# andreeaiana/manner

Measured on AMD Instinct MI355X. Metric: candidate news encoded+scored/sec, higher is better.
Workload: dtype f16; 1 GPU; configs[1]: CR-Module late fusion, MIND-small shape (65238-news pool), bert-base-uncased architectu~; modules=1, parallelism=dp1 (impressions sharded, no collective)

## Files before the change

### manner_amd/build.py

```python
from __future__ import annotations

import os
import subprocess
import sys
from concurrent.futures import ThreadPoolExecutor

PKG = os.path.dirname(os.path.abspath(__file__))
ROOT = os.path.dirname(PKG)
CSRC = os.path.join(PKG, "csrc")
LIB = os.path.join(PKG, "lib", "libmanner_hip.so")
SOURCES = ["gemm.hip", "rowops.hip", "attention.hip", "attention_d32.hip", "scoring.hip", "pool.hip", "entity.hip", "metrics.hip", "collate.hip", "cache.hip", "encoder.hip", "train.hip", "train_attn.hip", "wgrad.hip", "train_small.hip", "axis0.hip", "rows_f32.hip", "poly.hip", "caum.hip", "gru.hip", "mins.hip", "miner.hip", "aspect.hip", "debias.hip", "seqcls.hip", "tsne.hip"]
FLAGS = ["--offload-arch=gfx950", "-O3", "-std=c++17", "-fPIC", "-fno-gpu-rdc", "-Wall", "-Wno-unused-function",
         "-I" + os.path.join(ROOT, "include"), "-I" + CSRC]


def _newest(paths):
    return max(os.path.getmtime(p) for p in paths)


def build_library(force: bool = False, verbose: bool = True) -> str:
    hipcc = os.environ.get("HIPCC", "/opt/rocm/bin/hipcc")
    objdir = os.path.join(PKG, "lib", "obj")
    os.makedirs(objdir, exist_ok=True)
    if not all(os.path.exists(os.path.join(CSRC, f"gemm_w{nw}_asm.inc")) for nw in (8, 4)):
        subprocess.run([sys.executable, os.path.join(ROOT, "tools", "gen_gemm_w.py")], check=True, capture_output=True)
    headers = [os.path.join(CSRC, "common.h"), os.path.join(CSRC, "train_common.h"), os.path.join(CSRC, "row_head.h"), os.path.join(CSRC, "gemm_w4_asm.inc"), os.path.join(CSRC, "gemm_w8_asm.inc"), os.path.join(ROOT, "include", "manner_hip.h")]
    if not force and os.path.exists(LIB) and os.path.getmtime(LIB) >= _newest([os.path.join(CSRC, s) for s in SOURCES] + headers):
        return LIB
    jobs = []
    for s in SOURCES:
        src, obj = os.path.join(CSRC, s), os.path.join(objdir, s + ".o")
        if force or not os.path.exists(obj) or os.path.getmtime(obj) < _newest([src] + headers):
            jobs.append((src, obj))

    def cc(job):
        src, obj = job
        cmd = [hipcc] + FLAGS + ["-c", src, "-o", obj]
        r = subprocess.run(cmd, capture_output=True, text=True)
        return job, r

    with ThreadPoolExecutor(max_workers=min(4, max(1, len(jobs)))) as ex:
        for (src, obj), r in ex.map(cc, jobs):
            if verbose and (r.stdout or r.stderr):
                sys.stderr.write(r.stdout + r.stderr)
            if r.returncode:
                raise RuntimeError(f"hipcc failed on {src}")
    objs = [os.path.join(objdir, s + ".o") for s in SOURCES]
    if jobs or not os.path.exists(LIB):
        r = subprocess.run([hipcc, "--offload-arch=gfx950", "-shared", "-fPIC", "-o", LIB] + objs,
                           capture_output=True, text=True)
        if r.returncode:
            sys.stderr.write(r.stdout + r.stderr)
            raise RuntimeError("link of libmanner_hip.so failed")
    return LIB


if __name__ == "__main__":
    print(build_library(force="--force" in sys.argv))
```

### manner_amd/csrc/common.h

```cpp
#pragma once
#include <hip/hip_runtime.h>
#include <stddef.h>
#include <stdint.h>

#include "manner_hip.h"

typedef __bf16 bf16_t;
typedef __bf16 bf16x8 __attribute__((ext_vector_type(8)));
typedef __bf16 bf16x4 __attribute__((ext_vector_type(4)));
typedef _Float16 f16_t;
typedef _Float16 f16x8 __attribute__((ext_vector_type(8)));
typedef _Float16 f16x4 __attribute__((ext_vector_type(4)));
typedef short s16x4 __attribute__((ext_vector_type(4)));
typedef float f32x16 __attribute__((ext_vector_type(16)));
typedef float f32x4 __attribute__((ext_vector_type(4)));

#define LDS_PTR(p) ((__attribute__((address_space(3))) void*)(p))
#define GLOBAL_PTR(p) ((const __attribute__((address_space(1))) void*)(p))

namespace manner {

int fail(int code, const char* fmt, ...);

#define MANNER_HIP_TRY(expr)                                                            \
// ... 52 lines not shown
                EPI_GELU_GRAD = 9 ,
                EPI_BIAS_GELU_DUAL16 = 10 ,
                EPI_GELU_GRAD16 = 11  };
enum DType { DT_F32 = 0, DT_BF16 = 1, DT_F16 = 2 };
static inline bool is_16bit(DType d) { return d != DT_F32; }

template <typename T> struct E16;
template <> struct E16<bf16_t> {
  typedef bf16x8 v8; typedef bf16x4 v4;
  static constexpr DType dtype = DT_BF16;
  static __device__ __forceinline__ f32x4 mfma16(const v8& a, const v8& b, const f32x4& c) { return __builtin_amdgcn_mfma_f32_16x16x32_bf16(a, b, c, 0, 0, 0); }
  static __device__ __forceinline__ f32x16 mfma32(const v8& a, const v8& b, const f32x16& c) { return __builtin_amdgcn_mfma_f32_32x32x16_bf16(a, b, c, 0, 0, 0); }
};
template <> struct E16<f16_t> {
  typedef f16x8 v8; typedef f16x4 v4;
  static constexpr DType dtype = DT_F16;
  static __device__ __forceinline__ f32x4 mfma16(const v8& a, const v8& b, const f32x4& c) { return __builtin_amdgcn_mfma_f32_16x16x32_f16(a, b, c, 0, 0, 0); }
  static __device__ __forceinline__ f32x16 mfma32(const v8& a, const v8& b, const f32x16& c) { return __builtin_amdgcn_mfma_f32_32x32x16_f16(a, b, c, 0, 0, 0); }
};

int gemm_tn(DType in, DType out, Epilogue epi, const void* X, const void* W, const float* bias,
            const void* residual, void* Y, int64_t m_bound, int N, int K, const int* m_total,
            hipStream_t stream);

int gemm_tn_batched16(DType in, const void* X, const void* W, const float* bias, float* Y, int batch, int64_t xs, int64_t ws,
                      int64_t ys, int rows, int N, int K, const int* m_total, hipStream_t stream);

struct DlnFinalize { void* mr_out; int32_t* arrive; float eps; bool done; };
int gemm_tn_dln(DType dt, Epilogue epi, const void* X, const void* W, const float* bias, const float* vec, const void* mr,
                void* part, void* Y, int64_t m_bound, int N, int K, const int* m_total, hipStream_t stream, int64_t m_exact = -1,
                DlnFinalize* fin = nullptr);

int pool_logits_mfma(const float* x, const float* W, const float* bias, const float* query, int64_t R, int D, int Q,
                     float* logits, hipStream_t stream);

bool pool_fused_supported(int64_t B, int64_t S, int D, int Q);
size_t pool_fused_workspace_bytes(int D, int Q);
int pool_fused(const float* x, const float* W, const float* bias, const float* query, int64_t B, int64_t S, int D, int Q, float* out,
               void* workspace, size_t workspace_bytes, hipStream_t stream);

int lengths_and_offsets(const int64_t* mask, int64_t n_news, int64_t padded_len, int32_t* lens,
                        int32_t* cu , int32_t* m_total , int64_t m_bound,
                        int64_t expect_tokens, int32_t* status, hipStream_t stream, int max_len);
int embed_layernorm(DType out, const int64_t* ids, int64_t n_news, int64_t padded_len, const int32_t* cu,
                    const float* word, const float* pos, const float* type0, const float* gamma,
                    const float* beta, int H, float eps, int pos_offset, int vocab, int max_pos,
                    void* x, int32_t* status, hipStream_t stream);
int layernorm_rows(DType out, const float* pre, const float* gamma, const float* beta, int H, float eps,
                   void* x, int64_t m_bound, const int* m_total, hipStream_t stream);
int embed_raw(DType dt, const int64_t* ids, int64_t n_news, int64_t padded_len, const int32_t* cu, const float* word,
              const float* pos, const float* type0, int H, float eps, int pos_offset, int vocab, int max_pos,
              void* raw, void* mr, int32_t* status, hipStream_t stream);
__device__ __forceinline__ float2 dln_row_stats(const float2 (&v)[16], float inv_h, float eps) {
  float s1 = v[0].x, s2 = v[0].y;
#pragma unroll
  for (int g = 1; g < 16; ++g) { s1 += v[g].x; s2 += v[g].y; }
  const float mean = s1 * inv_h;
  const float var = fmaxf(fmaf(s2, inv_h, -(mean * mean)), 0.f);
  return float2{mean, 1.0f / sqrtf(var + eps)};
}
int dln_finalize(const void* part, int groups, int H, float eps, void* mr, int64_t m_bound, const int* m_total,
                 hipStream_t stream);
int gather_cls_ln(DType dt, const void* raw, const void* mr, const int32_t* cu, int64_t n_news, int H, const float* gamma,
                  const float* beta, void* dst, hipStream_t stream);
int fold_layernorm(DType dt, const float* w, const float* bias, const float* gamma, const float* beta, int N, int K, void* wf,
                   float* c1, float* c2, hipStream_t stream);
int scatter_hidden(DType in, DType out_dt, const void* x, const void* mr, const int32_t* cu, int64_t n_news, int64_t lp, int H,
                   const float* gamma, const float* beta, void* out, hipStream_t stream);
int split3_rows(DType dt, bool weight, const float* x, void* out, int K, int64_t rows, const int* m_total, hipStream_t stream);
int layernorm_rows_split(DType split_dt, const float* pre, const float* gamma, const float* beta, int H, float eps, float* x, void* a3,
                         int64_t m_bound, const int* m_total, hipStream_t stream);
int add_vectors(const float* a, const float* b, float* out, int n, hipStream_t stream);
int set_device_int(int32_t* p, int32_t value, hipStream_t stream);
int gather_cls(DType in, const void* x, const int32_t* cu, int64_t n_news, int H, float* out, hipStream_t stream);
int gather_cls_rows(DType dt, const void* x, const int32_t* cu, int64_t n_news, int H, void* dst, hipStream_t stream);
int convert_f32_to_16(DType dt, const float* src, void* dst, int64_t n, hipStream_t stream);

int attention_varlen(DType dt, const void* qkv, void* ctx, const int32_t* cu, int64_t n_news, int heads,
                     int H, int max_len, hipStream_t stream, void* split_out = nullptr, DType split_dt = DT_F32);

int attention_cls(DType dt, const void* qcls, const void* kv, void* ctx_cls, const int32_t* cu, int64_t n_news,
                  int heads, int H, hipStream_t stream);

int attention_varlen_d32(DType dt, const void* qkv, void* ctx, const int32_t* cu, int64_t n_news, int heads, int H, int max_len,
                         hipStream_t stream);
int attention_cls_d32(DType dt, const void* qcls, const void* kv, void* ctx_cls, const int32_t* cu, int64_t n_news, int heads, int H,
                      hipStream_t stream);

int launch_axis0_attention(const float* qkv, float* att, int64_t N, int64_t E, int D, int heads, bool train_tiles, hipStream_t stream);

int wlin_f32(bool tanh_act, const float* x, int ldx, const float* W, int ldw, const float* bias, int64_t R, int K, int O, float* y, int ldy,
             hipStream_t stream);
int wlin_dx_f32(const float* dy, int ldy, const float* W, int ldw, int64_t R, int K, int O, float* dx, float* wt, hipStream_t stream);

constexpr int LIN_ROWS_OT = 64;
int launch_lin_rows(bool tanh_act, const float* x, const float* W, int ldw, const float* b, const float* rowadd, int S, int64_t R, int K, int O, float* y,
                    int ldy, float* deriv, hipStream_t stream);
int launch_proj_rows(const float* x, int64_t xsb, int64_t xss, const int64_t* len, const float* W, const float* b, int S, int C, int64_t R, int K, int O,
                     float* gi, float* xs, hipStream_t stream);
int launch_dx_rows(const float* dy, int ldy, const float* W, int ldw, int64_t R, int K, int O, const float* add, const float* mul, float* dx,
                   hipStream_t stream);
constexpr int WGRAD_MAX_GROUPS = 16, WGRAD_GROUP_ROWS = 64;
int wgrad_rows_groups(int64_t R);
size_t wgrad_rows_part_floats(int64_t R, int K, int O);
int launch_wgrad_rows(const float* dy, int ldy, const float* x, int64_t R, int K, int O, float* part, float* dW, int ldo, hipStream_t stream);
int launch_wgrad_reduce(const float* part, int K, int O, int G, float* dW, int ldo, hipStream_t stream);
int launch_colsum_rows(const float* dy, int ldy, int64_t R, int O, float* db, hipStream_t stream);
int launch_transpose_tile(const float* in, int ldw, int O, int K, float* out, hipStream_t stream);

struct FloatBump {
  float* base;
  size_t off = 0;
  explicit FloatBump(void* p) : base(static_cast<float*>(p)) {}
  float* take(size_t n) {
    float* p = base ? base + off : nullptr;
    off += (n + 63) / 64 * 64;
    return p;
  }
};

}
```

### manner_amd/csrc/encoder.hip

```cpp
#include <stdarg.h>
#include <stdio.h>
#include <stdlib.h>

#include <vector>

#include "common.h"

namespace manner {

static thread_local char g_err[512] = "";

int fail(int code, const char* fmt, ...) {
  va_list ap;
  va_start(ap, fmt);
  vsnprintf(g_err, sizeof(g_err), fmt, ap);
  va_end(ap);
  return code;
}

struct LayerWeights {
  void* wqkv = nullptr;
  void* wo = nullptr;
  void* w1 = nullptr;
  void* w2 = nullptr;
  void* wqkv_f = nullptr;
  void* w1_f = nullptr;
  float *cq1 = nullptr, *cf1 = nullptr;
};
struct LayerParams {
  float *bqkv, *bo, *ln1g, *ln1b, *b1, *b2, *ln2g, *ln2b;
  float *cq2 = nullptr, *cf2 = nullptr, *bo_res = nullptr, *b2_res = nullptr;
};

}

struct manner_hip_encoder {
  manner_hip_encoder_config cfg;
  uint32_t precisions = 0;
  float *word = nullptr, *pos = nullptr, *type0 = nullptr, *embg = nullptr, *embb = nullptr;
  std::vector<manner::LayerParams> params;
  std::vector<manner::LayerWeights> w[5];
  int32_t* status = nullptr;
  static constexpr int ARRIVE_CAP = 4096;
  int32_t* arrive = nullptr;
  std::vector<void*> allocs;
  int n_streams = 2;
  bool defer_ln = false;
  static constexpr int MAX_STREAMS = 4;
  hipStream_t side[MAX_STREAMS] = {};
  hipEvent_t join_ev[MAX_STREAMS] = {};
  hipEvent_t phase_ev[MAX_STREAMS] = {};
  bool profiling = false;
  struct Span { hipEvent_t a, b; int cls; };
  std::vector<Span> spans;
  std::vector<hipEvent_t> free_events;
};

namespace manner {
namespace {

inline DType act_dtype(int prec) { return prec == MANNER_HIP_PREC_BF16 ? DT_BF16 : prec == MANNER_HIP_PREC_F16 ? DT_F16 : DT_F32; }
inline size_t act_bytes(int prec) { return (prec == MANNER_HIP_PREC_BF16 || prec == MANNER_HIP_PREC_F16) ? 2 : 4; }
inline bool is_x3(int prec) { return prec == MANNER_HIP_PREC_BF16X3 || prec == MANNER_HIP_PREC_F16X3; }
inline DType x3_dtype(int prec) { return prec == MANNER_HIP_PREC_F16X3 ? DT_F16 : DT_BF16; }

int dev_alloc(manner_hip_encoder* e, size_t bytes, void** out) {
  MANNER_HIP_TRY(hipMalloc(out, bytes));
  e->allocs.push_back(*out);
  return MANNER_HIP_OK;
}
int dev_copy_f32(manner_hip_encoder* e, const float* src, size_t n, float** out, hipStream_t s) {
  int rc = dev_alloc(e, n * sizeof(float), (void**)out);
  if (rc) return rc;
  MANNER_HIP_TRY(hipMemcpyAsync(*out, src, n * sizeof(float), hipMemcpyDeviceToDevice, s));
  return MANNER_HIP_OK;
}
int pack_matrix(int prec, const float* src, size_t n, void* dst, size_t elem_off, hipStream_t s) {
  if (prec == MANNER_HIP_PREC_BF16 || prec == MANNER_HIP_PREC_F16)
    return convert_f32_to_16(prec == MANNER_HIP_PREC_F16 ? DT_F16 : DT_BF16, src, static_cast<char*>(dst) + elem_off * 2, (int64_t)n, s);
  MANNER_HIP_TRY(hipMemcpyAsync(static_cast<float*>(dst) + elem_off, src, n * sizeof(float), hipMemcpyDeviceToDevice, s));
  return MANNER_HIP_OK;
}

struct ProfScope {
  manner_hip_encoder* e; hipStream_t s; hipEvent_t a = nullptr, b = nullptr; int cls;
  static hipEvent_t get(manner_hip_encoder* e) {
    hipEvent_t ev = nullptr;
    if (!e->free_events.empty()) { ev = e->free_events.back(); e->free_events.pop_back(); }
    else if (hipEventCreate(&ev) != hipSuccess) ev = nullptr;
    return ev;
  }
  ProfScope(manner_hip_encoder* enc, hipStream_t st, int c) : e(enc), s(st), cls(c) {
    if (!e->profiling) return;
    a = get(e); b = get(e);
    if (a && b) (void)hipEventRecord(a, s);
  }
  ~ProfScope() {
    if (!a || !b) return;
    (void)hipEventRecord(b, s);
    e->spans.push_back({a, b, cls});
  }
};

struct Workspace {
  int32_t *lens, *cu, *m_total;
  float* pre;
  void *x, *qkv, *ctx, *ffn;
  void *xcls, *qcls;
  void *mr_in, *mr_mid, *part;
  int32_t* arrive = nullptr;
  void* a3;
  void* a3h;
  void *acc_x, *acc_ctx, *acc_x1;
  int32_t* cls_total;
  int64_t cls_cap;
};

constexpr int64_t CLS_CAP = 16384;

size_t carve(const manner_hip_encoder* e, int64_t max_news, int64_t m_cap, int prec, char* base, Workspace* ws) {
  const size_t es = act_bytes(prec);
  const size_t H = e->cfg.hidden, I = e->cfg.intermediate;
  size_t off = 0;
  if (ws) { ws->a3 = nullptr; ws->a3h = nullptr; }
  auto take = [&](size_t bytes) { size_t o = off; off += (size_t)round_up((int64_t)bytes, 256); return base ? base + o : nullptr; };
  char* p;
  p = take((size_t)max_news * 4); if (ws) ws->lens = (int32_t*)p;
  p = take((size_t)(max_news + 1) * 4); if (ws) ws->cu = (int32_t*)p;
  p = take(256); if (ws) ws->m_total = (int32_t*)p;
  p = take((size_t)m_cap * H * 4); if (ws) ws->pre = (float*)p;
  p = take((size_t)m_cap * H * es); if (ws) ws->x = p;
  p = take((size_t)m_cap * 3 * H * es); if (ws) ws->qkv = p;
  p = take((size_t)m_cap * H * es); if (ws) ws->ctx = p;
  p = take((size_t)m_cap * I * es); if (ws) ws->ffn = p;
  const size_t n_pad = (size_t)round_up(max_news, 256);
  p = take(n_pad * H * es); if (ws) ws->xcls = p;
  p = take(n_pad * H * es); if (ws) ws->qcls = p;
  p = take((size_t)m_cap * 8); if (ws) ws->mr_in = p;
  p = take((size_t)m_cap * 8); if (ws) ws->mr_mid = p;
  p = take((size_t)m_cap * (H / 64) * 8); if (ws) ws->part = p;
  if (is_x3(prec)) {
    p = take((size_t)m_cap * 3 * (H > I ? H : I) * 2); if (ws) ws->a3 = p;
    p = take((size_t)m_cap * 3 * H * 2); if (ws) ws->a3h = p;
  }
  const int64_t cls_cap = m_cap < CLS_CAP ? m_cap : CLS_CAP;
  if (ws) ws->cls_cap = cls_cap;
  p = take((size_t)(cls_cap + 256) * H * es); if (ws) ws->acc_x = p;
  p = take((size_t)(cls_cap + 256) * H * es); if (ws) ws->acc_ctx = p;
  p = take((size_t)(cls_cap + 256) * H * es); if (ws) ws->acc_x1 = p;
  p = take(256); if (ws) ws->cls_total = (int32_t*)p;
  return off;
}

struct PhaseGuard {
  hipEvent_t ev; hipStream_t s; bool done = false;
  void mark() { if (ev && !done) { (void)hipEventRecord(ev, s); done = true; } }
  ~PhaseGuard() { mark(); }
};

int encode_chunk(manner_hip_encoder* e, const int64_t* ids, const int64_t* mask, int64_t n_news, int64_t lp,
                 int64_t m_bound, int64_t expect_tokens, int prec, void* out, const Workspace& ws, hipStream_t s,
                 hipEvent_t phase_mark = nullptr, int hidden_layers = -1, DType hidden_dt = DT_F32, int64_t cls_off = 0) {
  PhaseGuard phase{phase_mark, s};
  const manner_hip_encoder_config& c = e->cfg;
  const DType dt = act_dtype(prec);
  const int H = c.hidden, I = c.intermediate;
  int rc;
  {
    ProfScope ps(e, s, MANNER_HIP_PROF_LENGTHS);
    if ((rc = lengths_and_offsets(mask, n_news, lp, ws.lens, ws.cu, ws.m_total, m_bound, expect_tokens, e->status, s,
                                 MANNER_HIP_MAX_LEN_INFER))) return rc;
  }
  const int pos_offset = c.arch == MANNER_HIP_ARCH_ROBERTA ? c.pad_id + 1 : 0;
#define PROF_STEP(cls, call) { ProfScope ps(e, s, cls); if ((rc = (call))) return rc; }
  const size_t es = act_bytes(prec);
  if (is_16bit(dt) && e->defer_ln) {
    PROF_STEP(MANNER_HIP_PROF_EMBED, embed_raw(dt, ids, n_news, lp, ws.cu, e->word, e->pos, e->type0, H, c.ln_eps, pos_offset,
                                               c.vocab, c.max_pos, ws.x, ws.mr_in, e->status, s))
    const int groups = H / 64;
    for (int l = 0; l < c.layers; ++l) {
      const LayerWeights& w = e->w[prec][l];
      const LayerParams& p = e->params[l];
      const float* g_in = l == 0 ? e->embg : e->params[l - 1].ln2g;
      const float* b_in = l == 0 ? e->embb : e->params[l - 1].ln2b;
      if (l == hidden_layers) break;
      if (hidden_layers < 0 && l + 1 == c.layers) {
        const int64_t n_bound = round_up(n_news, 256);
        const int32_t* n_total = ws.m_total + 1;
        const char* wkv = static_cast<const char*>(w.wqkv_f) + (size_t)H * H * 2;
        PROF_STEP(MANNER_HIP_PROF_GEMM_QKV, gemm_tn_dln(dt, EPI_NORM, ws.x, wkv, p.cq2 + H, w.cq1 + H, ws.mr_in, nullptr, ws.qkv, m_bound, 2 * H, H, ws.m_total, s, expect_tokens))
        char* ax = static_cast<char*>(ws.acc_x) + (size_t)cls_off * H * es;
        char* actx = static_cast<char*>(ws.acc_ctx) + (size_t)cls_off * H * es;
        PROF_STEP(MANNER_HIP_PROF_GATHER, gather_cls_ln(dt, ws.x, ws.mr_in, ws.cu, n_news, H, g_in, b_in, ax, s))
        PROF_STEP(MANNER_HIP_PROF_CLS_TAIL, gemm_tn(dt, dt, EPI_BIAS, ax, w.wqkv, p.bqkv, nullptr, ws.qcls, n_bound, H, H, n_total, s))
        PROF_STEP(MANNER_HIP_PROF_ATTENTION, attention_cls(dt, ws.qcls, ws.qkv, actx, ws.cu, n_news, c.heads, H, s))
        break;
      }
      PROF_STEP(MANNER_HIP_PROF_GEMM_QKV, gemm_tn_dln(dt, EPI_NORM, ws.x, w.wqkv_f, p.cq2, w.cq1, ws.mr_in, nullptr, ws.qkv, m_bound, 3 * H, H, ws.m_total, s, expect_tokens))
      PROF_STEP(MANNER_HIP_PROF_ATTENTION, attention_varlen(dt, ws.qkv, ws.ctx, ws.cu, n_news, c.heads, H, (int)lp, s))
      const bool fan_in = ws.arrive && m_bound / 192 + 1 <= manner_hip_encoder::ARRIVE_CAP;
      DlnFinalize fin_mid{ws.mr_mid, fan_in ? ws.arrive : nullptr, c.ln_eps, false}, fin_in{ws.mr_in, fan_in ? ws.arrive : nullptr, c.ln_eps, false};
      PROF_STEP(MANNER_HIP_PROF_GEMM_OUT, gemm_tn_dln(dt, EPI_NRES, ws.ctx, w.wo, p.bo_res, g_in, ws.mr_in, ws.part, ws.x, m_bound, H, H, ws.m_total, s, expect_tokens, &fin_mid))
      if (!fin_mid.done) PROF_STEP(MANNER_HIP_PROF_LAYERNORM, dln_finalize(ws.part, groups, H, c.ln_eps, ws.mr_mid, m_bound, ws.m_total, s))
      if (l == 0) phase.mark();
      PROF_STEP(MANNER_HIP_PROF_GEMM_FFN1, gemm_tn_dln(dt, EPI_NORM_GELU, ws.x, w.w1_f, p.cf2, w.cf1, ws.mr_mid, nullptr, ws.ffn, m_bound, I, H, ws.m_total, s, expect_tokens))
      PROF_STEP(MANNER_HIP_PROF_GEMM_FFN2, gemm_tn_dln(dt, EPI_NRES, ws.ffn, w.w2, p.b2_res, p.ln1g, ws.mr_mid, ws.part, ws.x, m_bound, H, I, ws.m_total, s, expect_tokens, &fin_in))
      if (!fin_in.done) PROF_STEP(MANNER_HIP_PROF_LAYERNORM, dln_finalize(ws.part, groups, H, c.ln_eps, ws.mr_in, m_bound, ws.m_total, s))
    }
    if (hidden_layers >= 0) {
      const float* g = hidden_layers == 0 ? e->embg : e->params[hidden_layers - 1].ln2g;
      const float* b = hidden_layers == 0 ? e->embb : e->params[hidden_layers - 1].ln2b;
      PROF_STEP(MANNER_HIP_PROF_GATHER, scatter_hidden(dt, hidden_dt, ws.x, ws.mr_in, ws.cu, n_news, lp, H, g, b, out, s))
    }
    return MANNER_HIP_OK;
  }
  {
    ProfScope ps(e, s, MANNER_HIP_PROF_EMBED);
    if ((rc = embed_layernorm(dt, ids, n_news, lp, ws.cu, e->word, e->pos, e->type0, e->embg, e->embb, H, c.ln_eps,
                              pos_offset, c.vocab, c.max_pos, ws.x, e->status, s)))
      return rc;
  }
  const bool x3 = is_x3(prec);
  const DType xdt = x3_dtype(prec);
  auto gemm = [&](DType out_dt, Epilogue epi, const void* A, const void* Wm, const float* bias, const void* res, void* Y,
                  int64_t mb, int N, int K, const int* mt) -> int {
    if (!x3) return gemm_tn(dt, out_dt, epi, A, Wm, bias, res, Y, mb, N, K, mt, s);
    int r = split3_rows(xdt, false, static_cast<const float*>(A), ws.a3, K, mb, mt, s);
    if (r) return r;
    return gemm_tn(xdt, DT_F32, epi == EPI_BIAS_RES ? EPI_BIAS_RES_F32 : epi, ws.a3, Wm, bias, res, Y, mb, N, 3 * K, mt, s);
  };
  const int full_layers = hidden_layers >= 0 ? hidden_layers : c.layers - 1;
  if (x3) PROF_STEP(MANNER_HIP_PROF_LAYERNORM, split3_rows(xdt, false, static_cast<const float*>(ws.x), ws.a3h, H, m_bound, ws.m_total, s))
  for (int l = 0; l < full_layers && x3; ++l) {
    const LayerWeights& w = e->w[prec][l];
    const LayerParams& p = e->params[l];
    float* xf = static_cast<float*>(ws.x);
    PROF_STEP(MANNER_HIP_PROF_GEMM_QKV, gemm_tn(xdt, DT_F32, EPI_BIAS, ws.a3h, w.wqkv, p.bqkv, nullptr, ws.qkv, m_bound, 3 * H, 3 * H, ws.m_total, s))
    static const bool attn_valu = getenv("MANNER_HIP_ATTN_F32_VALU") != nullptr;
    if (attn_valu) {
      PROF_STEP(MANNER_HIP_PROF_ATTENTION, attention_varlen(dt, ws.qkv, ws.ctx, ws.cu, n_news, c.heads, H, (int)lp, s))
      PROF_STEP(MANNER_HIP_PROF_LAYERNORM, split3_rows(xdt, false, static_cast<const float*>(ws.ctx), ws.a3h, H, m_bound, ws.m_total, s))
    } else {
      PROF_STEP(MANNER_HIP_PROF_ATTENTION, attention_varlen(dt, ws.qkv, ws.ctx, ws.cu, n_news, c.heads, H, (int)lp, s, ws.a3h, xdt))
    }
    PROF_STEP(MANNER_HIP_PROF_GEMM_OUT, gemm_tn(xdt, DT_F32, EPI_BIAS_RES_F32, ws.a3h, w.wo, p.bo, ws.x, ws.pre, m_bound, H, 3 * H, ws.m_total, s))
    PROF_STEP(MANNER_HIP_PROF_LAYERNORM, layernorm_rows_split(xdt, ws.pre, p.ln1g, p.ln1b, H, c.ln_eps, xf, ws.a3h, m_bound, ws.m_total, s))
    if (l == 0) phase.mark();
    PROF_STEP(MANNER_HIP_PROF_GEMM_FFN1, gemm_tn(xdt, xdt, EPI_BIAS_GELU_SPLIT3, ws.a3h, w.w1, p.b1, nullptr, ws.a3, m_bound, I, 3 * H, ws.m_total, s))
    PROF_STEP(MANNER_HIP_PROF_GEMM_FFN2, gemm_tn(xdt, DT_F32, EPI_BIAS_RES_F32, ws.a3, w.w2, p.b2, ws.x, ws.pre, m_bound, H, 3 * I, ws.m_total, s))
    PROF_STEP(MANNER_HIP_PROF_LAYERNORM, layernorm_rows_split(xdt, ws.pre, p.ln2g, p.ln2b, H, c.ln_eps, xf, ws.a3h, m_bound, ws.m_total, s))
  }
  for (int l = 0; l < full_layers && !x3; ++l) {
    const LayerWeights& w = e->w[prec][l];
    const LayerParams& p = e->params[l];
    PROF_STEP(MANNER_HIP_PROF_GEMM_QKV, gemm(dt, EPI_BIAS, ws.x, w.wqkv, p.bqkv, nullptr, ws.qkv, m_bound, 3 * H, H, ws.m_total))
    PROF_STEP(MANNER_HIP_PROF_ATTENTION, attention_varlen(dt, ws.qkv, ws.ctx, ws.cu, n_news, c.heads, H, (int)lp, s))
    PROF_STEP(MANNER_HIP_PROF_GEMM_OUT, gemm(DT_F32, EPI_BIAS_RES, ws.ctx, w.wo, p.bo, ws.x, ws.pre, m_bound, H, H, ws.m_total))
    PROF_STEP(MANNER_HIP_PROF_LAYERNORM, layernorm_rows(dt, ws.pre, p.ln1g, p.ln1b, H, c.ln_eps, ws.x, m_bound, ws.m_total, s))
    if (l == 0) phase.mark();
    PROF_STEP(MANNER_HIP_PROF_GEMM_FFN1, gemm(dt, EPI_BIAS_GELU, ws.x, w.w1, p.b1, nullptr, ws.ffn, m_bound, I, H, ws.m_total))
    PROF_STEP(MANNER_HIP_PROF_GEMM_FFN2, gemm(DT_F32, EPI_BIAS_RES, ws.ffn, w.w2, p.b2, ws.x, ws.pre, m_bound, H, I, ws.m_total))
    PROF_STEP(MANNER_HIP_PROF_LAYERNORM, layernorm_rows(dt, ws.pre, p.ln2g, p.ln2b, H, c.ln_eps, ws.x, m_bound, ws.m_total, s))
  }
  if (hidden_layers >= 0) {
    PROF_STEP(MANNER_HIP_PROF_GATHER, scatter_hidden(dt, hidden_dt, ws.x, nullptr, ws.cu, n_news, lp, H, nullptr, nullptr, out, s))
    return MANNER_HIP_OK;
  }
  {
    const LayerWeights& w = e->w[prec][c.layers - 1];
    const LayerParams& p = e->params[c.layers - 1];
    const int64_t n_bound = round_up(n_news, 256);
    const int32_t* n_total = ws.m_total + 1;
    const char* wkv = static_cast<const char*>(w.wqkv) + (size_t)H * (x3 ? (size_t)3 * H * 2 : (size_t)H * es);
    if (x3)
      PROF_STEP(MANNER_HIP_PROF_GEMM_QKV, gemm_tn(xdt, DT_F32, EPI_BIAS, ws.a3h, wkv, p.bqkv + H, nullptr, ws.qkv, m_bound, 2 * H, 3 * H, ws.m_total, s))
    else
      PROF_STEP(MANNER_HIP_PROF_GEMM_QKV, gemm(dt, EPI_BIAS, ws.x, wkv, p.bqkv + H, nullptr, ws.qkv, m_bound, 2 * H, H, ws.m_total))
    char* ax = static_cast<char*>(ws.acc_x) + (size_t)cls_off * H * es;
// ... 125 lines not shown
  e->precisions = precisions;
  int rc = MANNER_HIP_OK;
  auto guard = [&](int r) { if (r && !rc) rc = r; return r == 0; };
  const size_t HH = (size_t)H * H, HI = (size_t)H * I;
  do {
    if (!guard(dev_copy_f32(e, weights[MANNER_HIP_W_WORD_EMB], (size_t)cfg->vocab * H, &e->word, s))) break;
    if (!guard(dev_copy_f32(e, weights[MANNER_HIP_W_POS_EMB], (size_t)cfg->max_pos * H, &e->pos, s))) break;
    if (!guard(dev_copy_f32(e, weights[MANNER_HIP_W_TYPE_EMB], (size_t)H, &e->type0, s))) break;
    if (!guard(dev_copy_f32(e, weights[MANNER_HIP_W_EMB_LN_G], H, &e->embg, s))) break;
    if (!guard(dev_copy_f32(e, weights[MANNER_HIP_W_EMB_LN_B], H, &e->embb, s))) break;
    if (!guard(dev_alloc(e, 256, (void**)&e->status))) break;
    if (hipMemsetAsync(e->status, 0, 256, s) != hipSuccess) { rc = fail(MANNER_HIP_E_RUNTIME, "memset failed"); break; }
    const size_t arrive_bytes = (size_t)manner_hip_encoder::MAX_STREAMS * manner_hip_encoder::ARRIVE_CAP * sizeof(int32_t);
    if (!guard(dev_alloc(e, arrive_bytes, (void**)&e->arrive))) break;
    if (hipMemsetAsync(e->arrive, 0, arrive_bytes, s) != hipSuccess) { rc = fail(MANNER_HIP_E_RUNTIME, "memset failed"); break; }
    if (const char* ev = getenv("MANNER_HIP_STREAMS")) {
      const int v = atoi(ev);
      e->n_streams = v < 1 ? 1 : (v > manner_hip_encoder::MAX_STREAMS ? manner_hip_encoder::MAX_STREAMS : v);
    }
    e->defer_ln = (precisions & ((1u << MANNER_HIP_PREC_BF16) | (1u << MANNER_HIP_PREC_F16))) && H % 256 == 0 && I % 256 == 0;
    if (const char* ev = getenv("MANNER_HIP_DEFER_LN")) e->defer_ln = e->defer_ln && atoi(ev) != 0;
    for (int i = 0; i < e->n_streams && !rc; ++i) {
      if ((i > 0 && hipStreamCreateWithFlags(&e->side[i], hipStreamNonBlocking) != hipSuccess) ||
          hipEventCreateWithFlags(&e->join_ev[i], hipEventDisableTiming) != hipSuccess ||
          hipEventCreateWithFlags(&e->phase_ev[i], hipEventDisableTiming) != hipSuccess)
        rc = fail(MANNER_HIP_E_RUNTIME, "encoder_create: side stream/event creation failed");
    }
    if (rc) break;
    e->params.resize(L);
    for (int p = 0; p < 5; ++p) if (precisions & (1u << p)) e->w[p].resize(L);
    for (int l = 0; l < L && !rc; ++l) {
      const float* const* wl = weights + MANNER_HIP_W_EMB_COUNT + l * MANNER_HIP_WL_COUNT;
      LayerParams& P = e->params[l];
      if (!guard(dev_alloc(e, 3 * (size_t)H * 4, (void**)&P.bqkv))) break;
      for (int j = 0; j < 3; ++j)
        if (hipMemcpyAsync(P.bqkv + j * H, wl[MANNER_HIP_WL_Q_B + 2 * j], H * 4, hipMemcpyDeviceToDevice, s) != hipSuccess) rc = fail(MANNER_HIP_E_RUNTIME, "bias copy failed");
      guard(dev_copy_f32(e, wl[MANNER_HIP_WL_AO_B], H, &P.bo, s));
      guard(dev_copy_f32(e, wl[MANNER_HIP_WL_ALN_G], H, &P.ln1g, s));
      guard(dev_copy_f32(e, wl[MANNER_HIP_WL_ALN_B], H, &P.ln1b, s));
      guard(dev_copy_f32(e, wl[MANNER_HIP_WL_FF1_B], I, &P.b1, s));
      guard(dev_copy_f32(e, wl[MANNER_HIP_WL_FF2_B], H, &P.b2, s));
      guard(dev_copy_f32(e, wl[MANNER_HIP_WL_OLN_G], H, &P.ln2g, s));
      guard(dev_copy_f32(e, wl[MANNER_HIP_WL_OLN_B], H, &P.ln2b, s));
      for (int p = 0; p < 4 && !rc; ++p) {
        if (is_x3(p) || !(precisions & (1u << p))) continue;
        const size_t es = act_bytes(p);
        LayerWeights& W = e->w[p][l];
        if (!guard(dev_alloc(e, 3 * HH * es, &W.wqkv))) break;
        if (!guard(dev_alloc(e, HH * es, &W.wo))) break;
        if (!guard(dev_alloc(e, HI * es, &W.w1))) break;
        if (!guard(dev_alloc(e, HI * es, &W.w2))) break;
        for (int j = 0; j < 3; ++j) guard(pack_matrix(p, wl[MANNER_HIP_WL_Q_W + 2 * j], HH, W.wqkv, j * HH, s));
        guard(pack_matrix(p, wl[MANNER_HIP_WL_AO_W], HH, W.wo, 0, s));
        guard(pack_matrix(p, wl[MANNER_HIP_WL_FF1_W], HI, W.w1, 0, s));
        guard(pack_matrix(p, wl[MANNER_HIP_WL_FF2_W], HI, W.w2, 0, s));
      }
      for (int p : {MANNER_HIP_PREC_BF16X3, MANNER_HIP_PREC_F16X3}) {
        if (!(precisions & (1u << p)) || rc) continue;
        const DType sdt = x3_dtype(p);
        LayerWeights& W = e->w[p][l];
        if (!guard(dev_alloc(e, 3 * HH * 6, &W.wqkv)) || !guard(dev_alloc(e, HH * 6, &W.wo)) ||
            !guard(dev_alloc(e, HI * 6, &W.w1)) || !guard(dev_alloc(e, HI * 6, &W.w2))) break;
        for (int j = 0; j < 3; ++j)
          guard(split3_rows(sdt, true, wl[MANNER_HIP_WL_Q_W + 2 * j], static_cast<char*>(W.wqkv) + (size_t)j * HH * 6, H, H, nullptr, s));
        guard(split3_rows(sdt, true, wl[MANNER_HIP_WL_AO_W], W.wo, H, H, nullptr, s));
        guard(split3_rows(sdt, true, wl[MANNER_HIP_WL_FF1_W], W.w1, H, I, nullptr, s));
        guard(split3_rows(sdt, true, wl[MANNER_HIP_WL_FF2_W], W.w2, I, H, nullptr, s));
      }
      if (e->defer_ln && !rc) {
        const float* g_in = l == 0 ? e->embg : e->params[l - 1].ln2g;
        const float* b_in = l == 0 ? e->embb : e->params[l - 1].ln2b;
        if (!guard(dev_alloc(e, 3 * (size_t)H * 4, (void**)&P.cq2)) || !guard(dev_alloc(e, (size_t)I * 4, (void**)&P.cf2))) break;
        if (!guard(dev_alloc(e, (size_t)H * 4, (void**)&P.bo_res)) || !guard(dev_alloc(e, (size_t)H * 4, (void**)&P.b2_res))) break;
        for (int p : {MANNER_HIP_PREC_BF16, MANNER_HIP_PREC_F16}) {
          if (!(precisions & (1u << p)) || rc) continue;
          const DType fdt = act_dtype(p);
          LayerWeights& W = e->w[p][l];
          if (!guard(dev_alloc(e, 3 * HH * 2, &W.wqkv_f)) || !guard(dev_alloc(e, HI * 2, &W.w1_f))) break;
          if (!guard(dev_alloc(e, 3 * (size_t)H * 4, (void**)&W.cq1)) || !guard(dev_alloc(e, (size_t)I * 4, (void**)&W.cf1))) break;
          for (int j = 0; j < 3; ++j)
            guard(fold_layernorm(fdt, wl[MANNER_HIP_WL_Q_W + 2 * j], wl[MANNER_HIP_WL_Q_B + 2 * j], g_in, b_in, H, H,
                                 static_cast<char*>(W.wqkv_f) + j * HH * 2, W.cq1 + j * H, P.cq2 + j * H, s));
          guard(fold_layernorm(fdt, wl[MANNER_HIP_WL_FF1_W], wl[MANNER_HIP_WL_FF1_B], P.ln1g, P.ln1b, I, H, W.w1_f, W.cf1, P.cf2, s));
        }
        guard(add_vectors(P.bo, b_in, P.bo_res, H, s));
        guard(add_vectors(P.b2, P.ln1b, P.b2_res, H, s));
      }
    }
    if (rc) break;
    if (hipStreamSynchronize(s) != hipSuccess) { rc = fail(MANNER_HIP_E_RUNTIME, "encoder_create: stream sync failed: %s", hipGetErrorString(hipGetLastError())); break; }
  } while (0);
  if (rc) { manner_hip_encoder_destroy(e); return rc; }
  *out = e;
  return MANNER_HIP_OK;
}

size_t manner_hip_encoder_workspace_bytes(manner_hip_encoder_t enc, int64_t max_news, int64_t max_tokens, int32_t precision) {
  if (!enc || max_news <= 0 || max_tokens <= 0 || precision < 0 || precision > 4) return 0;
  return enc->n_streams * carve(enc, max_news, round_up(max_tokens, 256), precision, nullptr, nullptr);
}

static int encode_impl(manner_hip_encoder_t enc, const int64_t* ids, const int64_t* mask, const int32_t* host_lengths,
                       int64_t n_news, int64_t padded_len, int32_t precision, void* out, void* workspace,
                       size_t workspace_bytes, manner_hip_stream_t stream, int hidden_layers, DType hidden_dt) {
  if (!enc) return fail(MANNER_HIP_E_INVALID, "encode_cls: null handle");
  if (n_news == 0) return MANNER_HIP_OK;
  if (!ids || !mask || !out || !workspace || n_news < 0) return fail(MANNER_HIP_E_INVALID, "encode_cls: null pointer");
  if (precision < 0 || precision > 4 || !(enc->precisions & (1u << precision))) return fail(MANNER_HIP_E_INVALID, "encode_cls: precision %d was not requested at encoder_create", precision);
  if (padded_len < 1 || padded_len > MANNER_HIP_MAX_LEN_INFER) return fail(MANNER_HIP_E_INVALID, "encode_cls: padded_len %lld outside [1, %d]", (long long)padded_len, MANNER_HIP_MAX_LEN_INFER);
  if ((uintptr_t)workspace % 256) return fail(MANNER_HIP_E_INVALID, "encode_cls: workspace must be 256-byte aligned");
  const int H = enc->cfg.hidden;
  const int ns = enc->profiling ? 1 : enc->n_streams;
  const size_t ws_each = (workspace_bytes / enc->n_streams) / 256 * 256;
  const size_t es = act_bytes(precision);
  const size_t per_tok = (size_t)H * 4 + ((size_t)5 * H + enc->cfg.intermediate) * es +
                         (is_x3(precision) ? (size_t)6 * (H > enc->cfg.intermediate ? H : enc->cfg.intermediate) + (size_t)6 * H : 0);
  int64_t m_cap = (int64_t)(ws_each / per_tok) / 256 * 256;
  int64_t n_cap = 0;
  while (m_cap >= 256) {
    n_cap = m_cap;
    if (n_cap > n_news) n_cap = n_news;
    if (carve(enc, n_cap, m_cap, precision, nullptr, nullptr) <= ws_each) break;
    m_cap -= 256;
  }
  if (m_cap < 256 || m_cap < padded_len) return fail(MANNER_HIP_E_WORKSPACE, "encode_cls: workspace of %zu bytes cannot hold one 256-token tile per stream", workspace_bytes);
  Workspace ws[manner_hip_encoder::MAX_STREAMS];
  for (int i = 0; i < ns; ++i) {
    carve(enc, n_cap, m_cap, precision, static_cast<char*>(workspace) + i * ws_each, &ws[i]);
    ws[i].arrive = enc->arrive + (size_t)i * manner_hip_encoder::ARRIVE_CAP;
  }
  hipStream_t s0 = (hipStream_t)stream;
  int forked = 0;
  auto join = [&]() -> int {
    for (int i = 1; i <= forked; ++i) {
      MANNER_HIP_TRY(hipEventRecord(enc->join_ev[i], enc->side[i]));
      MANNER_HIP_TRY(hipStreamWaitEvent(s0, enc->join_ev[i], 0));
    }
    forked = 0;
    return MANNER_HIP_OK;
  };
  struct Chunk { int64_t n0, cnt, m_bound, expect; };
  std::vector<Chunk> plan;
  for (int64_t n0 = 0; n0 < n_news;) {
    int64_t cnt = 0, m_bound, expect = -1;
    if (host_lengths) {
      int64_t tok = 0;
      while (n0 + cnt < n_news && cnt < n_cap) {
        const int64_t len = host_lengths[n0 + cnt];
        if (len < 1 || len > padded_len)
          return fail(MANNER_HIP_E_INVALID, "encode_cls: host_lengths[%lld]=%lld outside [1, padded_len]", (long long)(n0 + cnt), (long long)len);
        if (tok + len > m_cap) break;
        tok += len;
        ++cnt;
      }
      m_bound = round_up(tok, 256);
      expect = tok;
    } else {
      cnt = m_cap / padded_len;
      if (cnt > n_cap) cnt = n_cap;
      if (cnt > n_news - n0) cnt = n_news - n0;
      m_bound = round_up(cnt * padded_len, 256);
    }
    plan.push_back({n0, cnt, m_bound, expect});
    n0 += cnt;
  }
  const int n_chunks = (int)plan.size();
// ... 85 lines not shown
```

Before: 43850 candidates/s.

## Replace last-layer K/V projection with CLS-query-folded attention over raw rows

In the last encoder layer only the CLS query is needed, so instead of projecting K and V for every token, the CLS query is folded into the K weight (u = q·Wk^T) and attention scores are computed directly against the layer-normalised hidden rows. The softmax-weighted sum of the raw rows is then projected once through Wv per head. This removes the 2H-wide per-token K/V GEMM, at the cost of three new kernels, per-news scratch reused from the qkv buffer, and hi/lo split 16-bit MFMAs to keep precision. It applies only for H=768, 12 heads and padded length up to 96, and an environment variable disables it.

```diff
diff --git a/manner_amd/build.py b/manner_amd/build.py
--- a/manner_amd/build.py
+++ b/manner_amd/build.py
@@ -9,7 +9,7 @@
 ROOT = os.path.dirname(PKG)
 CSRC = os.path.join(PKG, "csrc")
 LIB = os.path.join(PKG, "lib", "libmanner_hip.so")
-SOURCES = ["gemm.hip", "rowops.hip", "attention.hip", "attention_d32.hip", "scoring.hip", "pool.hip", "entity.hip", "metrics.hip", "collate.hip", "cache.hip", "encoder.hip", "train.hip", "train_attn.hip", "wgrad.hip", "train_small.hip", "axis0.hip", "rows_f32.hip", "poly.hip", "caum.hip", "gru.hip", "mins.hip", "miner.hip", "aspect.hip", "debias.hip", "seqcls.hip", "tsne.hip"]
+SOURCES = ["gemm.hip", "rowops.hip", "attention.hip", "attention_d32.hip", "scoring.hip", "pool.hip", "entity.hip", "metrics.hip", "collate.hip", "cache.hip", "encoder.hip", "train.hip", "train_attn.hip", "wgrad.hip", "train_small.hip", "axis0.hip", "rows_f32.hip", "poly.hip", "caum.hip", "gru.hip", "mins.hip", "miner.hip", "aspect.hip", "debias.hip", "seqcls.hip", "tsne.hip", "cls_raw.hip"]
 FLAGS = ["--offload-arch=gfx950", "-O3", "-std=c++17", "-fPIC", "-fno-gpu-rdc", "-Wall", "-Wno-unused-function",
          "-I" + os.path.join(ROOT, "include"), "-I" + CSRC]
 
diff --git a/manner_amd/csrc/cls_raw.hip b/manner_amd/csrc/cls_raw.hip
--- /dev/null
+++ b/manner_amd/csrc/cls_raw.hip
@@ -0,0 +1,241 @@
+#include "common.h"
+
+namespace manner {
+namespace {
+
+constexpr int CR_H = 768, CR_HEADS = 12;
+constexpr int CR_COLS = 2 * CR_HEADS;
+constexpr int CR_ROWS = 32;
+constexpr int CR_LD = CR_H + 16;
+constexpr int CR_PLD = CR_ROWS + 8;
+constexpr size_t CR_U_ELEMS = (size_t)CR_COLS * CR_H, CR_Z_ELEMS = (size_t)CR_HEADS * CR_H;
+
+__global__ __launch_bounds__(256) void cls_transpose16_kernel(const uint16_t* __restrict__ w, uint16_t* __restrict__ wt, int n) {
+  __shared__ uint16_t tile[32][33];
+  const int c0 = blockIdx.y * 32, k0 = blockIdx.x * 32, tx = threadIdx.x & 31, ty = threadIdx.x >> 5;
+  for (int r = ty; r < 32; r += 8) tile[r][tx] = w[(size_t)(c0 + r) * n + k0 + tx];
+  __syncthreads();
+  for (int r = ty; r < 32; r += 8) wt[(size_t)(k0 + r) * n + c0 + tx] = tile[tx][r];
+}
+
+template <typename TE>
+__global__ __launch_bounds__(256) void cls_u_kernel(const TE* __restrict__ qcls, const TE* __restrict__ wkT, TE* __restrict__ u, int64_t first,
+                                                    int rows) {
+  using v8 = typename E16<TE>::v8;
+  const int lane = threadIdx.x & 63, i = lane & 15, g = lane >> 4, h = blockIdx.y;
+  const int r0 = blockIdx.x * 64 + (threadIdx.x >> 6) * 16;
+  if (r0 >= rows) return;
+  const int ra = min(r0 + i, rows - 1);
+  const TE* qp = qcls + (size_t)(first + ra) * CR_H + 64 * h + 8 * g;
+  const v8 a0 = *reinterpret_cast<const v8*>(qp), a1 = *reinterpret_cast<const v8*>(qp + 32);
+  const TE* wp = wkT + (size_t)i * CR_H + 64 * h + 8 * g;
+#pragma unroll 4
+  for (int nb = 0; nb < CR_H / 16; ++nb) {
+    const v8 b0 = *reinterpret_cast<const v8*>(wp + (size_t)nb * 16 * CR_H), b1 = *reinterpret_cast<const v8*>(wp + (size_t)nb * 16 * CR_H + 32);
+    f32x4 acc = {0.f, 0.f, 0.f, 0.f};
+    acc = E16<TE>::mfma16(a0, b0, acc);
+    acc = E16<TE>::mfma16(a1, b1, acc);
+#pragma unroll
+    for (int e = 0; e < 4; ++e) {
+      const int r = r0 + 4 * g + e;
+      if (r < rows) {
+        const TE hi = (TE)acc[e];
+        TE* up = u + (size_t)r * CR_U_ELEMS + (size_t)h * CR_H + 16 * nb + i;
+        up[0] = hi;
+        up[(size_t)CR_HEADS * CR_H] = (TE)(acc[e] - (float)hi);
+      }
+    }
+  }
+}
+
+template <typename TE>
+__global__ __launch_bounds__(256) void cls_rows_attn_kernel(const TE* __restrict__ raw, const float2* __restrict__ mr, const int32_t* __restrict__ cu,
+                                                            const TE* __restrict__ u, float* __restrict__ z, int64_t first) {
+  using v8 = typename E16<TE>::v8;
+  __shared__ __attribute__((aligned(16))) TE xs[CR_ROWS * CR_LD];
+  __shared__ float sc[CR_ROWS][CR_COLS + 1];
+  __shared__ __attribute__((aligned(16))) TE ph[16][CR_PLD], pl[16][CR_PLD];
+  __shared__ float m_run[16], l_run[16], alpha_s[16];
+  const int t = threadIdx.x, w = t >> 6, lane = t & 63, i = lane & 15, g = lane >> 4;
+  const int64_t n = first + blockIdx.x;
+  const int tok0 = cu[n], L = max(cu[n + 1] - tok0, 0);
+  const TE* un = u + (size_t)blockIdx.x * CR_U_ELEMS;
+  for (int k = t; k < 16 * CR_PLD; k += 256) { (&ph[0][0])[k] = (TE)0.f; (&pl[0][0])[k] = (TE)0.f; }
+  if (t < 16) { m_run[t] = -INFINITY; l_run[t] = 0.f; alpha_s[t] = 0.f; }
+  f32x4 acc[12];
+#pragma unroll
+  for (int b = 0; b < 12; ++b) acc[b] = f32x4{0.f, 0.f, 0.f, 0.f};
+  for (int r0 = 0; r0 < L; r0 += CR_ROWS) {
+    const int rows = min(CR_ROWS, L - r0);
+#pragma unroll
+    for (int it = 0; it < CR_ROWS * (CR_H / 8) / 256; ++it) {
+      const int p = t + 256 * it, j = p / (CR_H / 8), o = p - j * (CR_H / 8);
+      v8 out;
+      if (j < rows) {
+        const size_t row = (size_t)tok0 + r0 + j;
+        const v8 r = *reinterpret_cast<const v8*>(raw + row * CR_H + 8 * o);
+        const float2 ms = mr[row];
+#pragma unroll
+        for (int e = 0; e < 8; ++e) out[e] = (TE)(((float)r[e] - ms.x) * ms.y);
+      } else {
+#pragma unroll
+        for (int e = 0; e < 8; ++e) out[e] = (TE)0.f;
+      }
+      *reinterpret_cast<v8*>(&xs[j * CR_LD + 8 * o]) = out;
+    }
+    __syncthreads();
+    {
+      const int mb = w & 1, nbk = w >> 1;
+      if (16 * mb < rows) {
+        const int col = 16 * nbk + i;
+        const TE* up = un + (size_t)min(col, CR_COLS - 1) * CR_H + 8 * g;
+        const TE* xp = &xs[(16 * mb + i) * CR_LD + 8 * g];
+        f32x4 s = {0.f, 0.f, 0.f, 0.f};
+#pragma unroll 8
+        for (int ks = 0; ks < CR_H / 32; ++ks)
+          s = E16<TE>::mfma16(*reinterpret_cast<const v8*>(xp + 32 * ks), *reinterpret_cast<const v8*>(up + 32 * ks), s);
+        if (col < CR_COLS) {
+#pragma unroll
+          for (int e = 0; e < 4; ++e) sc[16 * mb + 4 * g + e][col] = s[e];
+        }
+      }
+    }
+    __syncthreads();
+#pragma unroll
+    for (int hh = 0; hh < 3; ++hh) {
+      const int h = 3 * w + hh;
+      const bool live = lane < rows;
+      const float s = live ? (sc[lane & (CR_ROWS - 1)][h] + sc[lane & (CR_ROWS - 1)][CR_HEADS + h]) * 0.125f : -INFINITY;
+      const float m_old = m_run[h];
+      const float mn = fmaxf(m_old, wmax(s));
+      const float p = live ? expf(s - mn) : 0.f;
+      const float psum = wsum(p);
+      if (lane < CR_ROWS) {
+        const int slot = 8 * (lane & 3) + (lane >> 2);
+        const TE hi = (TE)p;
+        ph[h][slot] = hi;
+        pl[h][slot] = (TE)(p - (float)hi);
+      }
+      if (lane == 0) {
+        const float alpha = expf(m_old - mn);
+        m_run[h] = mn;
+        l_run[h] = fmaf(l_run[h], alpha, psum);
+        alpha_s[h] = alpha;
+      }
+    }
+    __syncthreads();
+    {
+      const v8 a_hi = *reinterpret_cast<const v8*>(&ph[i][8 * g]), a_lo = *reinterpret_cast<const v8*>(&pl[i][8 * g]);
+      float al[4];
+#pragma unroll
+      for (int e = 0; e < 4; ++e) al[e] = alpha_s[4 * g + e];
+#pragma unroll
+      for (int b = 0; b < 12; ++b) {
+        const TE* xp = &xs[g * CR_LD + 192 * w + 16 * b + i];
+        v8 bx;
+#pragma unroll
+        for (int e = 0; e < 8; ++e) bx[e] = xp[4 * e * CR_LD];
+#pragma unroll
+        for (int e = 0; e < 4; ++e) acc[b][e] *= al[e];
+        acc[b] = E16<TE>::mfma16(a_hi, bx, acc[b]);
+        acc[b] = E16<TE>::mfma16(a_lo, bx, acc[b]);
+      }
+    }
+    __syncthreads();
+  }
+  __syncthreads();
+  float* zn = z + (size_t)blockIdx.x * CR_Z_ELEMS;
+#pragma unroll
+  for (int e = 0; e < 4; ++e) {
+    const int h = 4 * g + e;
+    if (h < CR_HEADS) {
+      const float l = l_run[h], inv = l > 0.f ? 1.0f / l : 0.f;
+#pragma unroll
+      for (int b = 0; b < 12; ++b) zn[(size_t)h * CR_H + 192 * w + 16 * b + i] = acc[b][e] * inv;
+    }
+  }
+}
+
+template <typename TE>
+__global__ __launch_bounds__(256) void cls_ctx_kernel(const float* __restrict__ z, const TE* __restrict__ wv, const float* __restrict__ c2v,
+                                                      TE* __restrict__ ctx, int rows) {
+  using v8 = typename E16<TE>::v8;
+  const int lane = threadIdx.x & 63, i = lane & 15, g = lane >> 4, h = blockIdx.y;
+  const int r0 = blockIdx.x * 64 + (threadIdx.x >> 6) * 16;
+  if (r0 >= rows) return;
+  const float* zp = z + (size_t)min(r0 + i, rows - 1) * CR_Z_ELEMS + (size_t)h * CR_H + 8 * g;
+  const TE* wp = wv + (size_t)(64 * h + i) * CR_H + 8 * g;
+  f32x4 acc[4];
+#pragma unroll
+  for (int b = 0; b < 4; ++b) acc[b] = f32x4{0.f, 0.f, 0.f, 0.f};
+#pragma unroll 4
+  for (int ks = 0; ks < CR_H / 32; ++ks) {
+    const f32x4 z0 = *reinterpret_cast<const f32x4*>(zp + 32 * ks), z1 = *reinterpret_cast<const f32x4*>(zp + 32 * ks + 4);
+    v8 a_hi, a_lo;
+#pragma unroll
+    for (int e = 0; e < 4; ++e) {
+      a_hi[e] = (TE)z0[e]; a_lo[e] = (TE)(z0[e] - (float)a_hi[e]);
+      a_hi[4 + e] = (TE)z1[e]; a_lo[4 + e] = (TE)(z1[e] - (float)a_hi[4 + e]);
+    }
+#pragma unroll
+    for (int b = 0; b < 4; ++b) {
+      const v8 bw = *reinterpret_cast<const v8*>(wp + (size_t)16 * b * CR_H + 32 * ks);
+      acc[b] = E16<TE>::mfma16(a_hi, bw, acc[b]);
+      acc[b] = E16<TE>::mfma16(a_lo, bw, acc[b]);
+    }
+  }
+#pragma unroll
+  for (int b = 0; b < 4; ++b) {
+    const int c = 64 * h + 16 * b + i;
+    const float bias = c2v[c];
+#pragma unroll
+    for (int e = 0; e < 4; ++e) {
+      const int r = r0 + 4 * g + e;
+      if (r < rows) ctx[(size_t)r * CR_H + c] = (TE)(acc[b][e] + bias);
+    }
+  }
+}
+
+template <typename TE>
+int launch_cls_rows(const void* raw, const void* mr, const int32_t* cu, const void* qcls, const void* wkT, const void* wv, const float* c2v,
+                    void* scratch, size_t scratch_bytes, void* ctx_cls, int64_t n_news, hipStream_t stream) {
+  const size_t per_news = CR_U_ELEMS * 2 + CR_Z_ELEMS * 4;
+  const int64_t cap = (int64_t)(scratch_bytes / per_news);
+  if (cap < 1) return fail(MANNER_HIP_E_WORKSPACE, "cls_rows_attention: scratch of %zu bytes holds no news", scratch_bytes);
+  TE* u = static_cast<TE*>(scratch);
+  float* z = reinterpret_cast<float*>(static_cast<char*>(scratch) + (size_t)cap * CR_U_ELEMS * 2);
+  for (int64_t first = 0; first < n_news; first += cap) {
+    const int rows = (int)(n_news - first < cap ? n_news - first : cap);
+    const dim3 gh((unsigned)((rows + 63) / 64), CR_HEADS), b(256);
+    hipLaunchKernelGGL(cls_u_kernel<TE>, gh, b, 0, stream, static_cast<const TE*>(qcls), static_cast<const TE*>(wkT), u, first, rows);
+    hipLaunchKernelGGL(cls_rows_attn_kernel<TE>, dim3((unsigned)rows), b, 0, stream, static_cast<const TE*>(raw), static_cast<const float2*>(mr), cu,
+                       static_cast<const TE*>(u), z, first);
+    hipLaunchKernelGGL(cls_ctx_kernel<TE>, gh, b, 0, stream, static_cast<const float*>(z), static_cast<const TE*>(wv), c2v,
+                       static_cast<TE*>(ctx_cls) + (size_t)first * CR_H, rows);
+    MANNER_LAUNCH_CHECK();
+  }
+  return MANNER_HIP_OK;
+}
+
+}
+
+bool cls_rows_supported(int heads, int H) { return H == CR_H && heads == CR_HEADS; }
+
+int cls_rows_pack(const void* wk_f, void* wk_t, int H, hipStream_t stream) {
+  if (H % 32) return fail(MANNER_HIP_E_INVALID, "cls_rows_pack: H=%d", H);
+  hipLaunchKernelGGL(cls_transpose16_kernel, dim3(H / 32, H / 32), dim3(256), 0, stream, static_cast<const uint16_t*>(wk_f),
+                     static_cast<uint16_t*>(wk_t), H);
+  MANNER_LAUNCH_CHECK();
+  return MANNER_HIP_OK;
+}
+
+int cls_rows_attention(DType dt, const void* raw, const void* mr, const int32_t* cu, const void* qcls, const void* wk_t, const void* wv_f,
+                       const float* c2v, void* scratch, size_t scratch_bytes, void* ctx_cls, int64_t n_news, int heads, int H,
+                       hipStream_t stream) {
+  if (!cls_rows_supported(heads, H) || !is_16bit(dt)) return fail(MANNER_HIP_E_INVALID, "cls_rows_attention: H=%d heads=%d dtype %d unsupported", H, heads, (int)dt);
+  if ((uintptr_t)scratch % 16) return fail(MANNER_HIP_E_INVALID, "cls_rows_attention: scratch must be 16-byte aligned");
+  if (dt == DT_F16) return launch_cls_rows<f16_t>(raw, mr, cu, qcls, wk_t, wv_f, c2v, scratch, scratch_bytes, ctx_cls, n_news, stream);
+  return launch_cls_rows<bf16_t>(raw, mr, cu, qcls, wk_t, wv_f, c2v, scratch, scratch_bytes, ctx_cls, n_news, stream);
+}
+
+}
diff --git a/manner_amd/csrc/common.h b/manner_amd/csrc/common.h
--- a/manner_amd/csrc/common.h
+++ b/manner_amd/csrc/common.h
@@ -158,6 +158,12 @@
 int attention_cls(DType dt, const void* qcls, const void* kv, void* ctx_cls, const int32_t* cu, int64_t n_news,
                   int heads, int H, hipStream_t stream);
 
+bool cls_rows_supported(int heads, int H);
+int cls_rows_pack(const void* wk_f, void* wk_t, int H, hipStream_t stream);
+int cls_rows_attention(DType dt, const void* raw, const void* mr, const int32_t* cu, const void* qcls, const void* wk_t, const void* wv_f,
+                       const float* c2v, void* scratch, size_t scratch_bytes, void* ctx_cls, int64_t n_news, int heads, int H,
+                       hipStream_t stream);
+
 int attention_varlen_d32(DType dt, const void* qkv, void* ctx, const int32_t* cu, int64_t n_news, int heads, int H, int max_len,
                          hipStream_t stream);
 int attention_cls_d32(DType dt, const void* qcls, const void* kv, void* ctx_cls, const int32_t* cu, int64_t n_news, int heads, int H,
diff --git a/manner_amd/csrc/encoder.hip b/manner_amd/csrc/encoder.hip
--- a/manner_amd/csrc/encoder.hip
+++ b/manner_amd/csrc/encoder.hip
@@ -25,6 +25,7 @@
   void* w2 = nullptr;
   void* wqkv_f = nullptr;
   void* w1_f = nullptr;
+  void* wk_t = nullptr;
   float *cq1 = nullptr, *cf1 = nullptr;
 };
 struct LayerParams {
@@ -106,6 +107,7 @@
   int32_t *lens, *cu, *m_total;
   float* pre;
   void *x, *qkv, *ctx, *ffn;
+  size_t qkv_bytes;
   void *xcls, *qcls;
   void *mr_in, *mr_mid, *part;
   int32_t* arrive = nullptr;
@@ -130,7 +132,7 @@
   p = take(256); if (ws) ws->m_total = (int32_t*)p;
   p = take((size_t)m_cap * H * 4); if (ws) ws->pre = (float*)p;
   p = take((size_t)m_cap * H * es); if (ws) ws->x = p;
-  p = take((size_t)m_cap * 3 * H * es); if (ws) ws->qkv = p;
+  p = take((size_t)m_cap * 3 * H * es); if (ws) { ws->qkv = p; ws->qkv_bytes = (size_t)m_cap * 3 * H * es; }
   p = take((size_t)m_cap * H * es); if (ws) ws->ctx = p;
   p = take((size_t)m_cap * I * es); if (ws) ws->ffn = p;
   const size_t n_pad = (size_t)round_up(max_news, 256);
@@ -188,12 +190,19 @@
         const int64_t n_bound = round_up(n_news, 256);
         const int32_t* n_total = ws.m_total + 1;
         const char* wkv = static_cast<const char*>(w.wqkv_f) + (size_t)H * H * 2;
-        PROF_STEP(MANNER_HIP_PROF_GEMM_QKV, gemm_tn_dln(dt, EPI_NORM, ws.x, wkv, p.cq2 + H, w.cq1 + H, ws.mr_in, nullptr, ws.qkv, m_bound, 2 * H, H, ws.m_total, s, expect_tokens))
+        const char* kv_env = getenv("MANNER_HIP_LAST_KV");
+        const bool rows_attn = w.wk_t && lp <= 96 && !(kv_env && atoi(kv_env) != 0);
+        if (!rows_attn)
+          PROF_STEP(MANNER_HIP_PROF_GEMM_QKV, gemm_tn_dln(dt, EPI_NORM, ws.x, wkv, p.cq2 + H, w.cq1 + H, ws.mr_in, nullptr, ws.qkv, m_bound, 2 * H, H, ws.m_total, s, expect_tokens))
         char* ax = static_cast<char*>(ws.acc_x) + (size_t)cls_off * H * es;
         char* actx = static_cast<char*>(ws.acc_ctx) + (size_t)cls_off * H * es;
         PROF_STEP(MANNER_HIP_PROF_GATHER, gather_cls_ln(dt, ws.x, ws.mr_in, ws.cu, n_news, H, g_in, b_in, ax, s))
         PROF_STEP(MANNER_HIP_PROF_CLS_TAIL, gemm_tn(dt, dt, EPI_BIAS, ax, w.wqkv, p.bqkv, nullptr, ws.qcls, n_bound, H, H, n_total, s))
-        PROF_STEP(MANNER_HIP_PROF_ATTENTION, attention_cls(dt, ws.qcls, ws.qkv, actx, ws.cu, n_news, c.heads, H, s))
+        if (rows_attn)
+          PROF_STEP(MANNER_HIP_PROF_ATTENTION, cls_rows_attention(dt, ws.x, ws.mr_in, ws.cu, ws.qcls, w.wk_t, wkv + (size_t)H * H * 2, p.cq2 + 2 * H, ws.qkv,
+                                                                  ws.qkv_bytes, actx, n_news, c.heads, H, s))
+        else
+          PROF_STEP(MANNER_HIP_PROF_ATTENTION, attention_cls(dt, ws.qcls, ws.qkv, actx, ws.cu, n_news, c.heads, H, s))
         break;
       }
       PROF_STEP(MANNER_HIP_PROF_GEMM_QKV, gemm_tn_dln(dt, EPI_NORM, ws.x, w.wqkv_f, p.cq2, w.cq1, ws.mr_in, nullptr, ws.qkv, m_bound, 3 * H, H, ws.m_total, s, expect_tokens))
@@ -485,6 +494,10 @@
             guard(fold_layernorm(fdt, wl[MANNER_HIP_WL_Q_W + 2 * j], wl[MANNER_HIP_WL_Q_B + 2 * j], g_in, b_in, H, H,
                                  static_cast<char*>(W.wqkv_f) + j * HH * 2, W.cq1 + j * H, P.cq2 + j * H, s));
           guard(fold_layernorm(fdt, wl[MANNER_HIP_WL_FF1_W], wl[MANNER_HIP_WL_FF1_B], P.ln1g, P.ln1b, I, H, W.w1_f, W.cf1, P.cf2, s));
+          if (l + 1 == L && cls_rows_supported(cfg->heads, H)) {
+            if (!guard(dev_alloc(e, HH * 2, &W.wk_t))) break;
+            guard(cls_rows_pack(static_cast<const char*>(W.wqkv_f) + HH * 2, W.wk_t, H, s));
+          }
         }
         guard(add_vectors(P.bo, b_in, P.bo_res, H, s));
         guard(add_vectors(P.b2, P.ln1b, P.b2_res, H, s));
```

Result: no change. 44210 candidates/s, median of 6 (+0.8%).
